# huangnengCSU/NanoSNP

Hardware: AMD Instinct MI355X
Metric: candidate SNP sites/sec (pileup encode + model fwd), 30x windows (higher is better)
Workload: dtype f32; 1 GPU; BASELINE configs[1]: pileup encode + PileupModel fwd, 1M synthetic 30x windows (G2) resident in HBM, batch=4096; batch=4096, windows_resident_per_gpu=1048576, streams=32, precision=fp32, parallelism=site-sharded x1, rooted gather of calls, world_size_observed=1, gather=torch

## Files before the change

### nanosnp_amd/csrc/nsnp_api.hip

```cpp
#include "nsnp_common.hpp"

#include <new>

extern "C" int nsnp_version(void) { return 101; }

extern "C" const char* nsnp_strerror(int code)
{
    switch (code) {
    case NSNP_OK: return "ok";
    case NSNP_EINVAL: return "invalid argument";
    case NSNP_ENOMEM: return "out of memory";
    case NSNP_EHIP: return "HIP runtime error";
    case NSNP_ENOWEIGHTS: return "weights not loaded";
    case NSNP_EARCH: return "device is not gfx950";
    case NSNP_ESHAPE: return "unsupported model dimensions";
    case NSNP_ENOTSUP: return "optional component unavailable (RCCL not found)";
    case NSNP_ECOMM: return "RCCL call failed";
    default: return "unknown error";
    }
}

static hipError_t g_create_err = hipSuccess;

extern "C" int nsnp_last_hip_error(const nsnp_ctx* ctx, const char** text)
{
    const hipError_t e = ctx ? ctx->last_err : g_create_err;
    if (text) *text = hipGetErrorString(e);
    return (int)e;
}

extern "C" int nsnp_ctx_create(int device, nsnp_ctx** out)
{
    if (!out) return NSNP_EINVAL;
    *out = nullptr;
    nsnp_ctx* ctx = new (std::nothrow) nsnp_ctx();
    if (!ctx) return NSNP_ENOMEM;
    memset((void*)ctx, 0, sizeof(*ctx));
    ctx->device = device;
    ctx->last_err = hipSuccess;
    ctx->chunk_sites = 32768;
    ctx->hap_chunk = 16384;
    ctx->precision = 0;
    ctx->hap_precision = 0;
    ctx->cat_precision = 0;
    ctx->cat_conv_lds = 1;
    ctx->cat_conv_pix2 = 1;
    ctx->hap_b3x = 1;
    ctx->tok_fused = 0;
    ctx->proj1_tiles = 4;
    ctx->fused_l1 = 1;
    ctx->l0_rs = 2;
    ctx->l1_rs = 1;
    ctx->l1_stagger = 0;
    ctx->head_rs = 1;
    ctx->rs_prio = 0;
    hipDeviceProp_t prop;
    hipError_t e = hipSetDevice(device);
    if (e == hipSuccess) e = hipGetDeviceProperties(&prop, device);
    if (e != hipSuccess) { g_create_err = e; delete ctx; return NSNP_EHIP; }
    if (strncmp(prop.gcnArchName, "gfx950", 6) != 0) { delete ctx; return NSNP_EARCH; }
    ctx->n_cu = prop.multiProcessorCount;
    *out = ctx;
    return NSNP_OK;
}

void nsnp_hap_free(nsnp_ctx* ctx);
int  nsnp_hap_reserve(nsnp_ctx* ctx);
void nsnp_cat_free(nsnp_ctx* ctx);
void nsnp_tok_free(nsnp_ctx* ctx);

constexpr size_t TIMER_MAX_PAIRS = 8192;

ScopedKernelTimer::ScopedKernelTimer(nsnp_ctx* c, int kernel, hipStream_t stream)
    : ctx(c), k(kernel), s(stream), stop_ev(nullptr), on(false)
{
    KernelTimer* t = c->timer;
    if (!t || !t->enabled || t->used[k] >= TIMER_MAX_PAIRS) return;
    if (t->used[k] == t->start[k].size()) {
        hipEvent_t a, b;
        if (hipEventCreate(&a) != hipSuccess) return;
        if (hipEventCreate(&b) != hipSuccess) { (void)hipEventDestroy(a); return; }
        t->start[k].push_back(a); t->stop[k].push_back(b);
    }
    const size_t i = t->used[k]++;
    (void)hipEventRecord(t->start[k][i], s);
    stop_ev = t->stop[k][i];
    on = true;
}
void ScopedKernelTimer::stop() { if (on) { (void)hipEventRecord(stop_ev, s); on = false; } }
ScopedKernelTimer::~ScopedKernelTimer() { stop(); }

extern "C" int nsnp_ctx_set_option(nsnp_ctx* ctx, const char* name, int64_t value)
{
    if (!ctx || !name) return NSNP_EINVAL;
    if (strcmp(name, "cat_precision") == 0) {
        if (value != 0 && value != 1 && value != 2) return NSNP_EINVAL;
        ctx->cat_precision = (int)value;
        return NSNP_OK;
    }
    if (strcmp(name, "tok_fused") == 0) {
        if (value != 0 && value != 1) return NSNP_EINVAL;
        ctx->tok_fused = (int)value;
        return NSNP_OK;
    }
    if (strcmp(name, "hap_b3x") == 0) {
        if (value != 0 && value != 1) return NSNP_EINVAL;
        ctx->hap_b3x = (int)value;
        return NSNP_OK;
    }
    if (strcmp(name, "cat_conv_pix2") == 0) {
        if (value != 0 && value != 1) return NSNP_EINVAL;
        ctx->cat_conv_pix2 = (int)value;
        return NSNP_OK;
    }
    if (strcmp(name, "cat_conv_lds") == 0) {
        if (value != 0 && value != 1) return NSNP_EINVAL;
        ctx->cat_conv_lds = (int)value;
        return NSNP_OK;
    }
    if (strcmp(name, "hap_precision") == 0) {
        if (value != 0 && value != 1 && value != 2) return NSNP_EINVAL;
        ctx->hap_precision = (int)value;
        return nsnp_hap_reserve(ctx);
    }
    if (strcmp(name, "hap_pass_sites") == 0) {
        if (value < 128 || value > 131072 || value % 128) return NSNP_EINVAL;
        const int64_t old = ctx->hap_chunk;
        ctx->hap_chunk = value;
        const int rc = nsnp_hap_reserve(ctx);
        if (rc) { ctx->hap_chunk = old; (void)nsnp_hap_reserve(ctx); }
        return rc;
    }
    if (strcmp(name, "pileup_precision") == 0) {
        if (value != 0 && value != 1 && value != 2) return NSNP_EINVAL;
        ctx->precision = (int)value;
        if (value == 2 && ctx->ws_h0 && ctx->ws_h0_floats < 192) return nsnp_ctx_reserve(ctx, ctx->chunk_sites);
        return NSNP_OK;
    }
    if (strcmp(name, "fused_l1") == 0) {
        if (value != 0 && value != 1) return NSNP_EINVAL;
        ctx->fused_l1 = (int)value;
        return NSNP_OK;
    }
    if (strcmp(name, "l0_register_stationary") == 0) {
        if (value != 0 && value != 1 && value != 2) return NSNP_EINVAL;
        ctx->l0_rs = (int)value;
        return NSNP_OK;
    }
    if (strcmp(name, "l1_register_stationary") == 0) {
        if (value != 0 && value != 1 && value != 2) return NSNP_EINVAL;
        ctx->l1_rs = (int)value;
        return NSNP_OK;
    }
    if (strcmp(name, "l0_input_weights_in_lds") == 0) {
        if (value != 0 && value != 1) return NSNP_EINVAL;
        ctx->l0_wx_lds = (int)value;
        return NSNP_OK;
    }
    if (strcmp(name, "static_priority") == 0) {
        if (value < 0 || value > 3) return NSNP_EINVAL;
        ctx->rs_prio = (int)value;
        return NSNP_OK;
    }
    if (strcmp(name, "head_split") == 0) {
        if (value != 0 && value != 1) return NSNP_EINVAL;
        ctx->head_rs = (int)value;
        return NSNP_OK;
    }
    if (strcmp(name, "l1_stagger") == 0) {
        if (value != 0 && value != 1) return NSNP_EINVAL;
        ctx->l1_stagger = (int)value;
        return NSNP_OK;
    }
    if (strcmp(name, "l1_site_groups") == 0) {
        if (value != 0 && value != 1 && value != 2 && value != 4) return NSNP_EINVAL;
        ctx->l1_rs_groups = (int)value;
        return NSNP_OK;
    }
    if (strcmp(name, "l0_site_groups") == 0) {
        if (value != 0 && value != 1 && value != 2 && value != 4) return NSNP_EINVAL;
        ctx->l0_rs_groups = (int)value;
        return NSNP_OK;
    }
    if (strcmp(name, "fused_waves") == 0) {
        if (value != 0 && value != 4 && value != 8 && value != 12) return NSNP_EINVAL;
        ctx->fused_waves = (int)value;
        return NSNP_OK;
    }
    if (strcmp(name, "proj1_tiles") == 0) {
        if (value < 1 || value > 64) return NSNP_EINVAL;
        ctx->proj1_tiles = (int)value;
        return NSNP_OK;
    }
    if (strcmp(name, "recurrence_waves") == 0) {
        if (value != 0 && value != 1 && value != 2 && value != 4 && value != 8) return NSNP_EINVAL;
        ctx->force_wpb = (int)value;
        return NSNP_OK;
    }
    return NSNP_EINVAL;
}

extern "C" int nsnp_ctx_enable_timing(nsnp_ctx* ctx, int enable)
{
    if (!ctx) return NSNP_EINVAL;
    if (!ctx->timer) {
        ctx->timer = new (std::nothrow) KernelTimer();
        if (!ctx->timer) return NSNP_ENOMEM;
        for (int k = 0; k < NSNP_K_COUNT; ++k) ctx->timer->used[k] = 0;
    }
    ctx->timer->enabled = enable != 0;
    return NSNP_OK;
}

extern "C" int nsnp_ctx_read_timing(nsnp_ctx* ctx, int kernel, double* total_ms, int64_t* launches)
{
    if (!ctx || kernel < 0 || kernel >= NSNP_K_COUNT || !total_ms || !launches) return NSNP_EINVAL;
    *total_ms = 0.0; *launches = 0;
    KernelTimer* t = ctx->timer;
    if (!t) return NSNP_OK;
    for (size_t i = 0; i < t->used[kernel]; ++i) {
        NSNP_HIP(ctx, hipEventSynchronize(t->stop[kernel][i]));
        float ms = 0.f;
        NSNP_HIP(ctx, hipEventElapsedTime(&ms, t->start[kernel][i], t->stop[kernel][i]));
        *total_ms += ms; ++*launches;
    }
    t->used[kernel] = 0;
    return NSNP_OK;
}

static void free_ws(nsnp_ctx* ctx)
{
    if (ctx->ws_h0) (void)hipFree(ctx->ws_h0);
    if (ctx->ws_xp1) (void)hipFree(ctx->ws_xp1);
    if (ctx->ws_h1c) (void)hipFree(ctx->ws_h1c);
    ctx->ws_h0 = ctx->ws_xp1 = ctx->ws_h1c = nullptr;
    ctx->ws_h0_floats = 0;
}

extern "C" int nsnp_ctx_destroy(nsnp_ctx* ctx)
{
    if (!ctx) return NSNP_EINVAL;
    (void)hipSetDevice(ctx->device);
    (void)hipDeviceSynchronize();
    free_ws(ctx);
    if (ctx->pw.arena) (void)hipFree(ctx->pw.arena);
    if (ctx->pw16.arena) (void)hipFree(ctx->pw16.arena);
    if (ctx->pw16.l1f_bias) (void)hipFree(ctx->pw16.l1f_bias);
    if (ctx->pwb3.arena) (void)hipFree(ctx->pwb3.arena);
    if (ctx->sel_tmp) (void)hipFree(ctx->sel_tmp);
    if (ctx->fil_tmp) (void)hipFree(ctx->fil_tmp);
    if (ctx->rec_tmp) (void)hipFree(ctx->rec_tmp);
    if (ctx->lab_tmp) (void)hipFree(ctx->lab_tmp);
    nsnp_tok_free(ctx);
    (void)nsnp_comm_destroy(ctx);
// ... 110 lines not shown
```

### nanosnp_amd/csrc/nsnp_common.hpp

```cpp
#pragma once

#include <hip/hip_runtime.h>
#include <stdint.h>
#include <stdlib.h>
#include <string.h>
#include <vector>

#include "nanosnp.h"

typedef float f32x4 __attribute__((ext_vector_type(4)));
typedef int   i32x4 __attribute__((ext_vector_type(4)));

#define NSNP_CDIV(a, b) (((a) + (b) - 1) / (b))

constexpr int PW = NSNP_PILEUP_WINDOW;
constexpr int PC = NSNP_PILEUP_CHANNELS;
constexpr int PH = 64;
constexpr int PG = 4 * PH;
constexpr int PCENTER = 16;
constexpr int PSTEPS1 = PCENTER + 1;


struct PileupWeightsDev {
    float* l0_whh[2];
    float* l0_wih[2];
    float* l0_wlast[2];
    void*  l0_wx[2];
    float* l1_wih[2];
    float* l1_bias[2];
    float* l1_bias_raw[2];
    float* l1_whh[2];
    float* proj_w;
    float* proj_b;
    float* dense_w;
    float* dense_b;
    float* head_w;
    float* head_b;
    float* arena;
    size_t arena_bytes;
    bool   loaded;
};

struct PileupWeightsF16 {
    void* l0_whh[2]; void* l0_wih_hi[2]; void* l0_wih_lo[2]; void* l1_wih[2]; void* l1_whh[2];
    void* l1f_hi[2]; void* l1f_lo[2]; float* l1f_bias;
    void* l0_wih_rs[2];
    void* l1_wih_rs[2]; void* l1_whh_rs[2];
    void* l0_whh_rs[2];
    void* proj_w; void* dense_w; void* head_w;
    void* arena; size_t arena_bytes; bool loaded;
};

struct PileupWeightsB3 {
    void* l0_whh[2]; void* l0_wih[2]; void* l1_wih[2]; void* l1_whh[2];
    void* proj_w; void* dense_w; void* head_w;
    float* proj_b; float* dense_b; float* head_b;
    void* arena; size_t arena_bytes; bool loaded;
};

struct HapWeightsDev;
struct CatWeightsDev;

enum { NSNP_K_L0 = 0, NSNP_K_PROJ1, NSNP_K_L1, NSNP_K_HEAD, NSNP_K_ENCODE, NSNP_K_HAPFEAT, NSNP_K_HAPLSTM, NSNP_K_CATCONV, NSNP_K_CAT,
       NSNP_K_COUNT };
struct KernelTimer {
    std::vector<hipEvent_t> start[NSNP_K_COUNT], stop[NSNP_K_COUNT];
    size_t used[NSNP_K_COUNT];
    bool enabled;
};

struct PostOut { uint8_t* gt_arg; uint8_t* zy_arg; float* gt_max; float* zy_max; };

struct nsnp_ctx {
    int device;
    int n_cu;
    hipError_t last_err;
    bool attr_set;
    bool attr_set_f16;
    bool attr_set_b3;
    int hap_b3x;
    int cat_conv_pix2;
    int cat_conv_lds;
    int cat_precision;
    int hap_precision;
    int precision;
    int fused_waves;
    int l0_rs;
    int l1_rs_groups;
    int l1_rs;
    int l0_rs_groups;
    int fused_l1;
    int proj1_tiles;
    int force_wpb;
    int l0_wx_lds;
    int rs_prio;
    int head_rs;
    int l1_stagger;
    int64_t chunk_sites;
    float*  ws_h0;
    int     ws_h0_floats;
    float*  ws_xp1;
    float*  ws_h1c;
    PileupWeightsDev pw;
    PileupWeightsF16 pw16;
    PileupWeightsB3 pwb3;
    HapWeightsDev* hw;
    void*  hap_ws; size_t hap_ws_bytes; int64_t hap_ws_chunk;
    int64_t hap_chunk;
    CatWeightsDev* cw;
    void*  cat_ws; size_t cat_ws_bytes;
    int64_t* sel_tmp; size_t sel_tmp_bytes;
    int64_t* fil_tmp; size_t fil_tmp_bytes;
    void* rec_tmp; size_t rec_tmp_bytes;
    void* lab_tmp; size_t lab_tmp_bytes;
    void* tok_ws; size_t tok_ws_bytes;
    void* ctg_ws; size_t ctg_ws_bytes;
    int tok_fused;
    bool af_cached; uint64_t af_bits, af_t; int af_k, af_mode; uint32_t af_table_words[128];
    bool af2_cached; uint64_t af2_bits, af2_t; int af2_k, af2_mode; uint32_t af2_table_words[128];
    KernelTimer* timer;
    void* comm; int comm_rank, comm_world;
    bool comm_borrowed;
};

struct ScopedKernelTimer {
    nsnp_ctx* ctx; int k; hipStream_t s; hipEvent_t stop_ev; bool on;
    ScopedKernelTimer(nsnp_ctx* c, int kernel, hipStream_t stream);
    void stop();
    ~ScopedKernelTimer();
};

#define NSNP_HIP(ctx, call)                                                        \
    do {                                                                           \
        hipError_t e_ = (call);                                                    \
        if (e_ != hipSuccess) { (ctx)->last_err = e_; return NSNP_EHIP; }          \
    } while (0)

typedef float (*nsnp_wfun)(const void* user, int row, int k);
void nsnp_pack_image(float* img, int n_tiles, int n_j4, nsnp_wfun f, const void* user);

int nsnp_ctx_need_xp1(nsnp_ctx* ctx);

int nsnp_pileup_forward_impl(nsnp_ctx* ctx, const int32_t* x, const int64_t* center_idx,
                             int64_t N, float* gt, float* zy, const PostOut* post, bool* post_written, hipStream_t s);
int nsnp_pileup_pack_weights(nsnp_ctx* ctx, const float* const* w);
int nsnp_pileup_forward_f16x3(nsnp_ctx* ctx, const int32_t* x, const int64_t* center_idx,
                              int64_t N, float* gt, float* zy, hipStream_t s);
int nsnp_pileup_pack_weights_f16(nsnp_ctx* ctx, const float* const* w);
int nsnp_pileup_forward_bf16x3(nsnp_ctx* ctx, const int32_t* x, const int64_t* center_idx, int64_t N, float* gt, float* zy,
                               const PostOut* post, hipStream_t s);
int nsnp_pileup_pack_weights_bf16(nsnp_ctx* ctx, const float* const* w);
```

### nanosnp_amd/csrc/nsnp_lstm_cell.hpp

```cpp
#pragma once

namespace nsnp_cell {

constexpr float LOG2E = 1.4426950408889634f;

static inline float lstm_gate_scale(int R) { return (R & 3) == 2 ? -2.0f * LOG2E : -LOG2E; }

__device__ __forceinline__ float cap64(float z) { return __builtin_amdgcn_fmed3f(z, -3.0e38f, 64.0f); }

__device__ __forceinline__ float lstm_cell(float zi, float zf, float zg, float zo, float c_prev, float& c_new)
{
    const float ei = __builtin_amdgcn_exp2f(zi);
    const float ef = __builtin_amdgcn_exp2f(zf);
    const float eo = __builtin_amdgcn_exp2f(zo);
    const float eg = __builtin_amdgcn_exp2f(cap64(zg));
    constexpr float K = -2.0f * LOG2E;
    const float tg = 1.0f + eg;
    const float ig = __builtin_fmaf(-K, eg, K) * __builtin_amdgcn_rcpf(__builtin_fmaf(ei, tg, tg));
    const float fg = __builtin_amdgcn_rcpf(1.0f + ef);
    const float cn = __builtin_fmaf(fg, c_prev, ig);
    const float ec = __builtin_amdgcn_exp2f(cap64(cn));
    c_new = cn;
    const float tc = 1.0f + ec;
    return (1.0f - ec) * __builtin_amdgcn_rcpf(__builtin_fmaf(eo, tc, tc));
}

}
```

### nanosnp_amd/csrc/pileup_forward.hip

```cpp
#include "nsnp_common.hpp"
#include "nsnp_lstm_cell.hpp"
#include "nsnp_devclock.hpp"
#include "nsnp_bf16.hpp"
#include <type_traits>

namespace {

constexpr float LOG2E = 1.4426950408889634f;

__device__ __forceinline__ f32x4 mfma4(float a, float b, f32x4 c)
{
    return __builtin_amdgcn_mfma_f32_16x16x4f32(a, b, c, 0, 0, 0);
}
__device__ __forceinline__ float sigmoid_f(float x)
{
    return __builtin_amdgcn_rcpf(1.0f + __builtin_amdgcn_exp2f(-LOG2E * x));
}
__device__ __forceinline__ float tanh_f(float x)
{
    return __builtin_fmaf(-2.0f, __builtin_amdgcn_rcpf(1.0f + __builtin_amdgcn_exp2f((2.0f * LOG2E) * x)), 1.0f);
}

__device__ __forceinline__ float lstm_cell(float zi, float zf, float zg, float zo, float& c)
{
// ... 770 lines not shown
        for (int k = 0; k < 2 * NSG; ++k) {
            const int64_t site = base_site + (tid >> 5) + 8 * k;
            const int64_t sc = site < N ? site : N - 1;
            sreg[k] = *reinterpret_cast<const f32x4*>(H0 + (sc * PW + t) * 128 + 4 * cid);
        }
    };
    auto store_h0 = [&](int buf) {
#pragma unroll
        for (int k = 0; k < 2 * NSG; ++k)
            *reinterpret_cast<f32x4*>(h0s + ((size_t)buf * NS + (tid >> 5) + 8 * k) * RS_H0ROW + 4 * slot) = sreg[k];
    };
    load_h0(dir ? PW - 1 : 0);
    store_h0(0);
    if (PSTEPS1 > 1) load_h0(dir ? PW - 2 : 1);
    __syncthreads();

    float c[NSG][4];
#pragma unroll
    for (int sg = 0; sg < NSG; ++sg)
#pragma unroll
        for (int u = 0; u < 4; ++u) c[sg][u] = 0.f;

    for (int s = 0; s < PSTEPS1; ++s) {
        const int t = dir ? PW - 1 - s : s;
        const int cur = s & 1;
        const float* h0b = h0s + (size_t)cur * NS * RS_H0ROW;
        const float* hrb = h1x + (size_t)(cur ^ 1) * NS * RS_XROW;
        float* hwb = h1x + (size_t)cur * NS * RS_XROW;
#pragma unroll
        for (int sg = 0; sg < NSG; ++sg) {
            const float* r0 = h0b + (size_t)(16 * sg + n) * RS_H0ROW + 4 * q;
            f32x4 acc[4];
#pragma unroll
            for (int u = 0; u < 4; ++u) acc[u] = lbias[(4 * wave + u) * 4 + q];
#pragma unroll
            for (int j = 0; j < 8; ++j) {
                if (sg == 0 && j == 2 && s + 1 < PSTEPS1) {
                    __builtin_amdgcn_sched_barrier(0);
                    store_h0(cur ^ 1);
                    __builtin_amdgcn_sched_barrier(0);
                }
                if (sg == 0 && j == 5 && s + 2 < PSTEPS1) {
                    __builtin_amdgcn_sched_barrier(0);
                    load_h0(dir ? t - 2 : t + 2);
                    __builtin_amdgcn_sched_barrier(0);
                }
                const f32x4 b4 = *reinterpret_cast<const f32x4*>(r0 + 64 * (j >> 2) + 16 * (j & 3));
#pragma unroll
                for (int e = 0; e < 4; ++e)
#pragma unroll
                    for (int u = 0; u < 4; ++u) acc[u] = mfma4(Wih[u][j][e], b4[e], acc[u]);
            }
            if (s > 0) {
                const float* r1 = hrb + (size_t)(16 * sg + n) * RS_XROW + 4 * q;
#pragma unroll
                for (int j = 0; j < 4; ++j) {
                    const f32x4 b4 = *reinterpret_cast<const f32x4*>(r1 + 16 * j);
#pragma unroll
                    for (int e = 0; e < 4; ++e)
#pragma unroll
                        for (int u = 0; u < 4; ++u) acc[u] = mfma4(Whh[u][j][e], b4[e], acc[u]);
                }
            }
            f32x4 hn;
#pragma unroll
            for (int u = 0; u < 4; ++u) {
                hn[u] = lstm_cell(acc[u][0], acc[u][1], acc[u][2], acc[u][3], c[sg][u]);
            }
            *reinterpret_cast<f32x4*>(hwb + (size_t)(16 * sg + n) * RS_XROW + 16 * wave + 4 * q) = hn;
        }
        lds_barrier();
    }
    const float* hfin = h1x + (size_t)((PSTEPS1 - 1) & 1) * NS * RS_XROW;
#pragma unroll
    for (int sg = 0; sg < NSG; ++sg) {
        const int64_t site = base_site + 16 * sg + n;
        if (site < N)
            *reinterpret_cast<f32x4*>(H1c + site * 128 + dir * 64 + q * 16 + 4 * wave) =
                *reinterpret_cast<const f32x4*>(hfin + (size_t)(16 * sg + n) * RS_XROW + 16 * wave + 4 * q);
    }
    NSNP_DEVCLK_STOP(1)
}

__global__ __launch_bounds__(256) void k_pileup_head(
    const float* __restrict__ H1c, int64_t N,
    const float* __restrict__ proj_w, const float* __restrict__ proj_b,
    const float* __restrict__ dense_w, const float* __restrict__ dense_b,
    const float* __restrict__ head_w, const float* __restrict__ head_b,
    float* __restrict__ gt_prob, float* __restrict__ zy_prob)
{
    const int tid = threadIdx.x, lane = tid & 63, wave = tid >> 6;
    const int q = lane >> 4;
    const int64_t site = ((int64_t)blockIdx.x * 4 + wave) * 16 + (lane & 15);
    const bool live = site < N;
    const int64_t sc = live ? site : N - 1;
    const f32x4* __restrict__ hin = reinterpret_cast<const f32x4*>(H1c + sc * 128 + q * 16);
    float b[32];
#pragma unroll
    for (int v = 0; v < 4; ++v) {
        const f32x4 a = hin[v], bb = hin[16 + v];
#pragma unroll
        for (int e = 0; e < 4; ++e) { b[4 * v + e] = a[e]; b[16 + 4 * v + e] = bb[e]; }
    }
    f32x4 ap[8];
    {
        const f32x4* pb = reinterpret_cast<const f32x4*>(proj_b);
#pragma unroll
        for (int i = 0; i < 8; ++i) ap[i] = pb[i * 64 + lane];
        wave_gemm<8, 8, 0, 8>(reinterpret_cast<const f32x4*>(proj_w), lane, b, ap);
    }
    float b2[32];
#pragma unroll
    for (int i = 0; i < 8; ++i)
#pragma unroll
        for (int g = 0; g < 4; ++g) b2[4 * i + g] = ap[i][g];
    f32x4 ad[16];
    {
        const f32x4* db = reinterpret_cast<const f32x4*>(dense_b);
#pragma unroll
        for (int i = 0; i < 16; ++i) ad[i] = db[i * 64 + lane];
        wave_gemm<16, 8, 0, 8>(reinterpret_cast<const f32x4*>(dense_w), lane, b2, ad);
    }
    float b3[64];
#pragma unroll
    for (int i = 0; i < 16; ++i)
#pragma unroll
        for (int g = 0; g < 4; ++g) b3[4 * i + g] = tanh_f(ad[i][g]);
    f32x4 ah[2];
    {
        const f32x4* hb = reinterpret_cast<const f32x4*>(head_b);
        ah[0] = hb[lane]; ah[1] = hb[64 + lane];
        wave_gemm2x16(reinterpret_cast<const f32x4*>(head_w), lane, b3, ah);
    }
    const float NEG = -3.0e38f;
    float g0[4], g1[4];
#pragma unroll
    for (int g = 0; g < 4; ++g) {
        g0[g] = ah[0][g];
        const bool is_gt = (q == 0) || (q == 1 && g == 0);
        g1[g] = is_gt ? ah[1][g] : NEG;
    }
    float mx = fmaxf(fmaxf(fmaxf(g0[0], g0[1]), fmaxf(g0[2], g0[3])), fmaxf(fmaxf(g1[0], g1[1]), fmaxf(g1[2], g1[3])));
    mx = fmaxf(mx, __shfl_xor(mx, 16));
    mx = fmaxf(mx, __shfl_xor(mx, 32));
    float e0[4], e1[4], sum = 0.f;
#pragma unroll
    for (int g = 0; g < 4; ++g) {
        e0[g] = __expf(g0[g] - mx);
        e1[g] = g1[g] > -1.0e38f ? __expf(g1[g] - mx) : 0.f;
        sum += e0[g] + e1[g];
    }
    sum += __shfl_xor(sum, 16);
    sum += __shfl_xor(sum, 32);
    const float z1 = ah[1][1], z2 = ah[1][2], z3 = ah[1][3];
    const float zm = fmaxf(z1, fmaxf(z2, z3));
    const float ez1 = __expf(z1 - zm), ez2 = __expf(z2 - zm), ez3 = __expf(z3 - zm);
    const float zs = ez1 + ez2 + ez3;
    if (live) {
        float* gp = gt_prob + site * NSNP_GT_CLASSES;
#pragma unroll
        for (int g = 0; g < 4; ++g) gp[4 * q + g] = e0[g] / sum;
        if (q == 0) {
#pragma unroll
            for (int g = 0; g < 4; ++g) gp[16 + g] = e1[g] / sum;
        }
        if (q == 1) {
// ... 235 lines not shown
    for (int t = 0; t < 16; ++t) {
        const int layer = t / 8, kind = t % 4;
        const size_t cols = kind == 0 ? (layer ? 2 * PH : PC) : (kind == 1 ? PH : 1);
        scaled[t].resize((size_t)4 * PH * cols);
        for (int r = 0; r < 4 * PH; ++r) {
            const float f = (r / PH == 2) ? -2.0f * LOG2E : -LOG2E;
            for (size_t k = 0; k < cols; ++k) scaled[t][r * cols + k] = f * w[t][r * cols + k];
        }
        ws[t] = scaled[t].data();
    }
    for (int d = 0; d < 2; ++d) {
        const float* const* l0 = ws + d * 4;
        const float* const* l1 = ws + 8 + d * 4;
        MatRef m;
        m = MatRef{l0[1], PH, nullptr, nullptr};  nsnp_pack_image(h_l0_whh[d], 16, 4, f_whh, &m);
        m = MatRef{l0[0], PC, nullptr, nullptr};  nsnp_pack_image(h_l0_wih[d], 16, 1, f_wih0, &m);
        for (int tile = 0; tile < 16; ++tile)
            for (int lane = 0; lane < 64; ++lane) {
                const int tr = gate_row(16 * tile + (lane & 15)), kq = lane >> 4;
                float v = 0.f;
                if (kq < 2) v = l0[0][tr * PC + 16 + kq];
                else if (kq == 2) v = l0[2][tr] + l0[3][tr];
                h_l0_wlast[d][tile * 64 + lane] = v;
            }
        pack_b3(reinterpret_cast<uint16_t*>(h_l0_wx[d]), 16, 1, [&](int row, int, int q, int j) {
            const int k = 8 * q + j, tr = gate_row(row);
            return k < PC ? l0[0][tr * PC + k] : (k == PC ? l0[2][tr] + l0[3][tr] : 0.f);
        });
        m = MatRef{l1[0], 2 * PH, nullptr, nullptr};  nsnp_pack_image(h_l1_wih[d], 16, 8, f_wih1, &m);
        for (int tile = 0; tile < 16; ++tile)
            for (int lane = 0; lane < 64; ++lane)
                for (int g = 0; g < 4; ++g) {
                    const int tr = gate_row(16 * tile + 4 * (lane >> 4) + g);
                    h_l1_b[d][(tile * 64 + lane) * 4 + g] = l1[2][tr] + l1[3][tr];
                    h_l1_braw[d][(tile * 64 + lane) * 4 + g] = w[8 + d * 4 + 2][tr] + w[8 + d * 4 + 3][tr];
                }
        m = MatRef{l1[1], PH, nullptr, nullptr};  nsnp_pack_image(h_l1_whh[d], 16, 4, f_whh, &m);
    }
    {
        MatRef m{w[16], 128, nullptr, nullptr};  nsnp_pack_image(h_proj, 8, 8, f_proj, &m);
        for (int tile = 0; tile < 8; ++tile) for (int lane = 0; lane < 64; ++lane) for (int g = 0; g < 4; ++g)
            h_pb[(tile * 64 + lane) * 4 + g] = w[17][16 * tile + 4 * (lane >> 4) + g];
        MatRef md{w[18], 128, nullptr, nullptr}; nsnp_pack_image(h_dense, 16, 8, f_dense, &md);
        for (int tile = 0; tile < 16; ++tile) for (int lane = 0; lane < 64; ++lane) for (int g = 0; g < 4; ++g)
            h_db[(tile * 64 + lane) * 4 + g] = w[19][16 * tile + 4 * (lane >> 4) + g];
        HeadRef hr{w[20], w[22]};  nsnp_pack_image(h_head, 2, 16, f_head, &hr);
        for (int tile = 0; tile < 2; ++tile) for (int lane = 0; lane < 64; ++lane) for (int g = 0; g < 4; ++g) {
            const int row = 16 * tile + 4 * (lane >> 4) + g;
            h_hb[(tile * 64 + lane) * 4 + g] = row < 21 ? w[21][row] : (row < 24 ? w[23][row - 21] : 0.f);
        }
    }
    if (pw.arena && pw.arena_bytes != total * sizeof(float)) { (void)hipFree(pw.arena); pw.arena = nullptr; }
    if (!pw.arena) {
        NSNP_HIP(ctx, hipMalloc((void**)&pw.arena, total * sizeof(float)));
        pw.arena_bytes = total * sizeof(float);
    }
    NSNP_HIP(ctx, hipMemcpy(pw.arena, host.data(), total * sizeof(float), hipMemcpyHostToDevice));
    auto dev = [&](const float* hp) { return pw.arena + (hp - host.data()); };
    for (int d = 0; d < 2; ++d) {
        pw.l0_whh[d] = dev(h_l0_whh[d]); pw.l0_wih[d] = dev(h_l0_wih[d]); pw.l0_wlast[d] = dev(h_l0_wlast[d]);
        pw.l0_wx[d] = dev(h_l0_wx[d]);
        pw.l1_wih[d] = dev(h_l1_wih[d]); pw.l1_bias[d] = dev(h_l1_b[d]); pw.l1_bias_raw[d] = dev(h_l1_braw[d]); pw.l1_whh[d] = dev(h_l1_whh[d]);
    }
    pw.proj_w = dev(h_proj); pw.proj_b = dev(h_pb); pw.dense_w = dev(h_dense); pw.dense_b = dev(h_db);
    pw.head_w = dev(h_head); pw.head_b = dev(h_hb);
    pw.loaded = true;
    return NSNP_OK;
}

static int set_lds_attr_once(nsnp_ctx* ctx)
{
    if (ctx->attr_set) return NSNP_OK;
    NSNP_HIP(ctx, hipFuncSetAttribute((const void*)k_pileup_l0<8>, hipFuncAttributeMaxDynamicSharedMemorySize, L0_LDS_BYTES));
    NSNP_HIP(ctx, hipFuncSetAttribute((const void*)k_pileup_l0<4>, hipFuncAttributeMaxDynamicSharedMemorySize, L0_LDS_BYTES));
    NSNP_HIP(ctx, hipFuncSetAttribute((const void*)k_pileup_l0<2>, hipFuncAttributeMaxDynamicSharedMemorySize, L0_LDS_BYTES));
    NSNP_HIP(ctx, hipFuncSetAttribute((const void*)k_pileup_l0<1>, hipFuncAttributeMaxDynamicSharedMemorySize, L0_LDS_BYTES));
    NSNP_HIP(ctx, hipFuncSetAttribute((const void*)k_pileup_proj1, hipFuncAttributeMaxDynamicSharedMemorySize, P1_LDS_BYTES));
    NSNP_HIP(ctx, hipFuncSetAttribute((const void*)k_pileup_l1<8>, hipFuncAttributeMaxDynamicSharedMemorySize, L1_LDS_BYTES));
    NSNP_HIP(ctx, hipFuncSetAttribute((const void*)k_pileup_l1<4>, hipFuncAttributeMaxDynamicSharedMemorySize, L1_LDS_BYTES));
    NSNP_HIP(ctx, hipFuncSetAttribute((const void*)k_pileup_l1<2>, hipFuncAttributeMaxDynamicSharedMemorySize, L1_LDS_BYTES));
    NSNP_HIP(ctx, hipFuncSetAttribute((const void*)k_pileup_l1<1>, hipFuncAttributeMaxDynamicSharedMemorySize, L1_LDS_BYTES));
    NSNP_HIP(ctx, hipFuncSetAttribute((const void*)k_pileup_l1_rs4<1>, hipFuncAttributeMaxDynamicSharedMemorySize, rs4_l1_lds_bytes(1)));
    NSNP_HIP(ctx, hipFuncSetAttribute((const void*)k_pileup_l1_rs4<2>, hipFuncAttributeMaxDynamicSharedMemorySize, rs4_l1_lds_bytes(2)));
    NSNP_HIP(ctx, hipFuncSetAttribute((const void*)k_pileup_l1_rs32<4, true>, hipFuncAttributeMaxDynamicSharedMemorySize, rs32_l1_lds_bytes(4)));
    NSNP_HIP(ctx, hipFuncSetAttribute((const void*)k_pileup_l1_rs32<2, true>, hipFuncAttributeMaxDynamicSharedMemorySize, rs32_l1_lds_bytes(2)));
    NSNP_HIP(ctx, hipFuncSetAttribute((const void*)k_pileup_l1_rs32<4, false>, hipFuncAttributeMaxDynamicSharedMemorySize, rs32_l1_lds_bytes(4)));
    NSNP_HIP(ctx, hipFuncSetAttribute((const void*)k_pileup_l1_rs32<2, false>, hipFuncAttributeMaxDynamicSharedMemorySize, rs32_l1_lds_bytes(2)));
    ctx->attr_set = true;
    return NSNP_OK;
}

int nsnp_pileup_forward_impl(nsnp_ctx* ctx, const int32_t* x, const int64_t* center_idx,
                             int64_t N, float* gt, float* zy, const PostOut* post, bool* post_written, hipStream_t s)
{
    if (!ctx->pw.loaded) return NSNP_ENOWEIGHTS;
    if (N == 0) return NSNP_OK;
    int rc = set_lds_attr_once(ctx);
    if (rc) return rc;
    if (!ctx->ws_h0) { rc = nsnp_ctx_reserve(ctx, ctx->chunk_sites); if (rc) return rc; }
    const PileupWeightsDev& pw = ctx->pw;
    for (int64_t base = 0; base < N; base += ctx->chunk_sites) {
        const int64_t n = (N - base < ctx->chunk_sites) ? N - base : ctx->chunk_sites;
        const int32_t* xc = center_idx ? x : x + base * (PW * PC);
        const int64_t* cc = center_idx ? center_idx + base : nullptr;
        const int64_t waves_total = NSNP_CDIV(n, 16) * 2;
        int wpb = 8;
        while (wpb > 1 && waves_total / wpb < (int64_t)ctx->n_cu / 2) wpb >>= 1;
        if (ctx->force_wpb) wpb = ctx->force_wpb;
        const dim3 g_rec((unsigned)NSNP_CDIV(n, 16 * wpb), 2);
        if (ctx->l0_rs == 2) {
            ScopedKernelTimer tm(ctx, NSNP_K_L0, s);
            hipLaunchKernelGGL(k_pileup_l0_rsx, dim3((unsigned)NSNP_CDIV(n, 16), 2), dim3(256), 0, s, xc, cc, n,
                               pw.l0_whh[0], pw.l0_whh[1], (const __bf16*)pw.l0_wx[0], (const __bf16*)pw.l0_wx[1], ctx->ws_h0);
        } else if (ctx->l0_rs) {
            ScopedKernelTimer tm(ctx, NSNP_K_L0, s);
            int nsg = 1;
            if (ctx->l0_rs_groups) nsg = ctx->l0_rs_groups;
#define LAUNCH_RS(G) hipLaunchKernelGGL(k_pileup_l0_rs32<G>, dim3((unsigned)NSNP_CDIV(n, 16 * G), 2), dim3(256), 0, s, xc, cc, n, \
                           pw.l0_whh[0], pw.l0_whh[1], pw.l0_wih[0], pw.l0_wih[1], pw.l0_wlast[0], pw.l0_wlast[1], ctx->ws_h0)
            if (ctx->l0_wx_lds && nsg == 1)
                hipLaunchKernelGGL((k_pileup_l0_rs32<1, true>), dim3((unsigned)NSNP_CDIV(n, 16), 2), dim3(256), 0, s, xc, cc, n,
                                   pw.l0_whh[0], pw.l0_whh[1], pw.l0_wih[0], pw.l0_wih[1], pw.l0_wlast[0], pw.l0_wlast[1], ctx->ws_h0);
            else
            if (nsg == 4) LAUNCH_RS(4); else if (nsg == 2) LAUNCH_RS(2); else LAUNCH_RS(1);
#undef LAUNCH_RS
        } else
        { ScopedKernelTimer tm(ctx, NSNP_K_L0, s);
#define LAUNCH_L0(W) hipLaunchKernelGGL(k_pileup_l0<W>, g_rec, dim3(64 * W), L0_LDS_BYTES, s, xc, cc, n, \
                           pw.l0_whh[0], pw.l0_whh[1], pw.l0_wih[0], pw.l0_wih[1], pw.l0_wlast[0], pw.l0_wlast[1], ctx->ws_h0)
        if (wpb == 8) LAUNCH_L0(8); else if (wpb == 4) LAUNCH_L0(4); else if (wpb == 2) LAUNCH_L0(2); else LAUNCH_L0(1);
#undef LAUNCH_L0
        }
        if (ctx->l1_rs == 1) {
            ScopedKernelTimer tm(ctx, NSNP_K_L1, s);
            int g1 = 1;
            if (ctx->l1_rs_groups == 1 || ctx->l1_rs_groups == 2) g1 = ctx->l1_rs_groups;
#define LAUNCH_R4(G) hipLaunchKernelGGL(k_pileup_l1_rs4<G>, dim3((unsigned)NSNP_CDIV(n, 16 * G), 2), dim3(256), rs4_l1_lds_bytes(G), s, \
                           ctx->ws_h0, n, pw.l1_wih[0], pw.l1_wih[1], pw.l1_whh[0], pw.l1_whh[1], pw.l1_bias[0], pw.l1_bias[1], ctx->ws_h1c)
            if (g1 == 2) LAUNCH_R4(2); else LAUNCH_R4(1);
#undef LAUNCH_R4
        } else if (ctx->l1_rs == 2) {
            ScopedKernelTimer tm(ctx, NSNP_K_L1, s);
            int g1 = NSNP_CDIV(n, 64) * 2 >= (int64_t)ctx->n_cu ? 4 : 2;
            if (ctx->l1_rs_groups) g1 = ctx->l1_rs_groups;
#define LAUNCH_R1(G) hipLaunchKernelGGL((k_pileup_l1_rs32<G, ST>), dim3((unsigned)NSNP_CDIV(n, 16 * G), 2), dim3(512), rs32_l1_lds_bytes(G), s, \
                           ctx->ws_h0, n, pw.l1_wih[0], pw.l1_wih[1], pw.l1_whh[0], pw.l1_whh[1], pw.l1_bias[0], pw.l1_bias[1], ctx->ws_h1c)
            if (ctx->l1_stagger) { constexpr bool ST = true; if (g1 == 4) LAUNCH_R1(4); else LAUNCH_R1(2); }
            else { constexpr bool ST = false; if (g1 == 4) LAUNCH_R1(4); else LAUNCH_R1(2); }
#undef LAUNCH_R1
        } else {
        { const int rx = nsnp_ctx_need_xp1(ctx); if (rx) return rx; }
        const int64_t n_rt = NSNP_CDIV(n * PSTEPS1, 16);
        int64_t gp = NSNP_CDIV(n_rt, 16 * (int64_t)ctx->proj1_tiles);
        if (gp > ctx->n_cu) gp = ctx->n_cu;
        if (gp < 1) gp = 1;
        { ScopedKernelTimer tm(ctx, NSNP_K_PROJ1, s);
        hipLaunchKernelGGL(k_pileup_proj1, dim3((unsigned)gp, 2), dim3(1024), P1_LDS_BYTES, s, ctx->ws_h0, n,
                           pw.l1_wih[0], pw.l1_wih[1], pw.l1_bias[0], pw.l1_bias[1], ctx->ws_xp1); }
        { ScopedKernelTimer tm(ctx, NSNP_K_L1, s);
#define LAUNCH_L1(W) hipLaunchKernelGGL(k_pileup_l1<W>, g_rec, dim3(64 * W), L1_LDS_BYTES, s, ctx->ws_xp1, n, \
                           pw.l1_whh[0], pw.l1_whh[1], ctx->ws_h1c)
        if (wpb == 8) LAUNCH_L1(8); else if (wpb == 4) LAUNCH_L1(4); else if (wpb == 2) LAUNCH_L1(2); else LAUNCH_L1(1);
#undef LAUNCH_L1
        }
        }
        ScopedKernelTimer tm_head(ctx, NSNP_K_HEAD, s);
        if (ctx->head_rs) {
            int64_t gh = NSNP_CDIV(n, 16);
            if (gh > 2 * (int64_t)ctx->n_cu) gh = 2 * (int64_t)ctx->n_cu;
            const PostOut po = post ? *post : PostOut{nullptr, nullptr, nullptr, nullptr};
            hipLaunchKernelGGL(k_pileup_head_rs, dim3((unsigned)gh), dim3(512), 0, s, ctx->ws_h1c, n,
                               pw.proj_w, pw.proj_b, pw.dense_w, pw.dense_b, pw.head_w, pw.head_b,
                               gt + base * NSNP_GT_CLASSES, zy + base * NSNP_ZY_CLASSES,
                               po.gt_arg ? po.gt_arg + base : nullptr, po.gt_arg ? po.zy_arg + base : nullptr,
                               po.gt_arg ? po.gt_max + base : nullptr, po.gt_arg ? po.zy_max + base : nullptr);
            if (post_written) *post_written = po.gt_arg != nullptr;
        } else
        hipLaunchKernelGGL(k_pileup_head, dim3((unsigned)NSNP_CDIV(n, 64)), dim3(256), 0, s, ctx->ws_h1c, n,
                           pw.proj_w, pw.proj_b, pw.dense_w, pw.dense_b, pw.head_w, pw.head_b,
                           gt + base * NSNP_GT_CLASSES, zy + base * NSNP_ZY_CLASSES);
    }
    NSNP_HIP(ctx, hipGetLastError());
    return NSNP_OK;
}

NSNP_DEVCLK_READER(nsnp_devclk_read_pileup)

extern "C" int nsnp_pileup_postprocess(nsnp_ctx* ctx, const float* gt_prob, const float* zy_prob,
                                       const int32_t* x, int64_t N, uint8_t* gt_arg, uint8_t* zy_arg,
                                       float* gt_max, float* zy_max, int32_t* depth, void* stream)
{
    if (!ctx || N < 0 || (N > 0 && (!gt_prob || !zy_prob || !gt_arg || !zy_arg || !gt_max || !zy_max || (depth && !x)))) return NSNP_EINVAL;
    if (N == 0) return NSNP_OK;
    hipLaunchKernelGGL(k_pileup_post, dim3((unsigned)NSNP_CDIV(N, 256)), dim3(256), 0, (hipStream_t)stream,
                       gt_prob, zy_prob, x, N, gt_arg, zy_arg, gt_max, zy_max, depth);
    NSNP_HIP(ctx, hipGetLastError());
    return NSNP_OK;
}
```

Baseline: 20.54 million sites/s.

## Add woven L1 LSTM kernel overlapping next-step projection with cell math

```diff
diff --git a/nanosnp_amd/csrc/nsnp_api.hip b/nanosnp_amd/csrc/nsnp_api.hip
--- a/nanosnp_amd/csrc/nsnp_api.hip
+++ b/nanosnp_amd/csrc/nsnp_api.hip
@@ -52,6 +52,7 @@
     ctx->l0_rs = 2;
     ctx->l1_rs = 1;
     ctx->l1_stagger = 0;
+    ctx->l1_weave = 1;
     ctx->head_rs = 1;
     ctx->rs_prio = 0;
     hipDeviceProp_t prop;
@@ -170,6 +171,11 @@
     if (strcmp(name, "l1_stagger") == 0) {
         if (value != 0 && value != 1) return NSNP_EINVAL;
         ctx->l1_stagger = (int)value;
+        return NSNP_OK;
+    }
+    if (strcmp(name, "l1_weave") == 0) {
+        if (value != 0 && value != 1) return NSNP_EINVAL;
+        ctx->l1_weave = (int)value;
         return NSNP_OK;
     }
     if (strcmp(name, "l1_site_groups") == 0) {
diff --git a/nanosnp_amd/csrc/nsnp_common.hpp b/nanosnp_amd/csrc/nsnp_common.hpp
--- a/nanosnp_amd/csrc/nsnp_common.hpp
+++ b/nanosnp_amd/csrc/nsnp_common.hpp
@@ -96,6 +96,7 @@
     int rs_prio;
     int head_rs;
     int l1_stagger;
+    int l1_weave;
     int64_t chunk_sites;
     float*  ws_h0;
     int     ws_h0_floats;
diff --git a/nanosnp_amd/csrc/nsnp_lstm_cell.hpp b/nanosnp_amd/csrc/nsnp_lstm_cell.hpp
--- a/nanosnp_amd/csrc/nsnp_lstm_cell.hpp
+++ b/nanosnp_amd/csrc/nsnp_lstm_cell.hpp
@@ -25,4 +25,45 @@
     return (1.0f - ec) * __builtin_amdgcn_rcpf(__builtin_fmaf(eo, tc, tc));
 }
 
+struct CellSlices { float ei[4], ef[4], eo[4], eg[4], t[4], d[4], m[4], fg[4]; };
+constexpr int CELL_SLICES = 80;
+
+template <int I, typename Z4>
+__device__ __forceinline__ void lstm_cell_slice(CellSlices& w, const Z4 (&z)[4], float (&c)[4], Z4& h)
+{
+    static_assert(I >= 0 && I < CELL_SLICES, "slice index");
+    constexpr int st = I >> 2, u = I & 3;
+    constexpr float K = -2.0f * LOG2E;
+    if constexpr (st == 0) w.ei[u] = __builtin_amdgcn_exp2f(z[u][0]);
+    else if constexpr (st == 1) w.ef[u] = __builtin_amdgcn_exp2f(z[u][1]);
+    else if constexpr (st == 2) w.eo[u] = __builtin_amdgcn_exp2f(z[u][3]);
+    else if constexpr (st == 3) w.t[u] = cap64(z[u][2]);
+    else if constexpr (st == 4) w.eg[u] = __builtin_amdgcn_exp2f(w.t[u]);
+    else if constexpr (st == 5) w.t[u] = 1.0f + w.eg[u];
+    else if constexpr (st == 6) w.d[u] = __builtin_fmaf(w.ei[u], w.t[u], w.t[u]);
+    else if constexpr (st == 7) w.d[u] = __builtin_amdgcn_rcpf(w.d[u]);
+    else if constexpr (st == 8) w.m[u] = __builtin_fmaf(-K, w.eg[u], K);
+    else if constexpr (st == 9) w.m[u] = w.m[u] * w.d[u];
+    else if constexpr (st == 10) w.fg[u] = 1.0f + w.ef[u];
+    else if constexpr (st == 11) w.fg[u] = __builtin_amdgcn_rcpf(w.fg[u]);
+    else if constexpr (st == 12) c[u] = __builtin_fmaf(w.fg[u], c[u], w.m[u]);
+    else if constexpr (st == 13) w.t[u] = cap64(c[u]);
+    else if constexpr (st == 14) w.eg[u] = __builtin_amdgcn_exp2f(w.t[u]);
+    else if constexpr (st == 15) w.t[u] = 1.0f + w.eg[u];
+    else if constexpr (st == 16) w.d[u] = __builtin_fmaf(w.eo[u], w.t[u], w.t[u]);
+    else if constexpr (st == 17) w.d[u] = __builtin_amdgcn_rcpf(w.d[u]);
+    else if constexpr (st == 18) w.m[u] = 1.0f - w.eg[u];
+    else h[u] = w.m[u] * w.d[u];
+    if constexpr (st == 0) asm volatile("" : "+v"(w.ei[u]));
+    else if constexpr (st == 1) asm volatile("" : "+v"(w.ef[u]));
+    else if constexpr (st == 2) asm volatile("" : "+v"(w.eo[u]));
+    else if constexpr (st == 4 || st == 14) asm volatile("" : "+v"(w.eg[u]));
+    else if constexpr (st == 3 || st == 5 || st == 13 || st == 15) asm volatile("" : "+v"(w.t[u]));
+    else if constexpr (st == 6 || st == 7 || st == 16 || st == 17) asm volatile("" : "+v"(w.d[u]));
+    else if constexpr (st == 8 || st == 9 || st == 18) asm volatile("" : "+v"(w.m[u]));
+    else if constexpr (st == 10 || st == 11) asm volatile("" : "+v"(w.fg[u]));
+    else if constexpr (st == 12) asm volatile("" : "+v"(c[u]));
+    else { float v = h[u]; asm volatile("" : "+v"(v)); h[u] = v; }
 }
+
+}
diff --git a/nanosnp_amd/csrc/pileup_forward.hip b/nanosnp_amd/csrc/pileup_forward.hip
--- a/nanosnp_amd/csrc/pileup_forward.hip
+++ b/nanosnp_amd/csrc/pileup_forward.hip
@@ -876,6 +876,186 @@
     NSNP_DEVCLK_STOP(1)
 }
 
+constexpr int rs4w_l1_lds_bytes() { return rs4_l1_lds_bytes(1) + 4 * 4 * 2 * 64 * 16; }
+
+template <int... I, class F>
+__device__ __forceinline__ void static_for_seq(std::integer_sequence<int, I...>, F&& f) { (f(std::integral_constant<int, I>{}), ...); }
+template <int N, class F>
+__device__ __forceinline__ void static_for(F&& f) { static_for_seq(std::make_integer_sequence<int, N>{}, f); }
+
+template <int CELL_PER_GAP, int CELL_FIRST_GAP>
+__global__ __launch_bounds__(256, 2) void k_pileup_l1_rs4w(
+    const float* __restrict__ H0, int64_t N,
+    const float* __restrict__ wih0, const float* __restrict__ wih1,
+    const float* __restrict__ whh0, const float* __restrict__ whh1,
+    const float* __restrict__ bias0, const float* __restrict__ bias1,
+    float* __restrict__ H1c)
+{
+    extern __shared__ f32x4 lds[];
+    float* const h0s = reinterpret_cast<float*>(lds);
+    float* const h1x = h0s + 2 * 16 * RS_H0ROW;
+    f32x4* const lbias = reinterpret_cast<f32x4*>(h1x + 2 * 16 * RS_XROW);
+    f32x4* const lwhh = lbias + 64;
+    const int dir = blockIdx.y;
+    const int tid = threadIdx.x, lane = tid & 63, wave = tid >> 6;
+    const int n = lane & 15, q = lane >> 4;
+    NSNP_DEVCLK_START
+    const int64_t base_site = (int64_t)blockIdx.x * 16;
+
+    f32x4 Wih[4][8], Whh[4][2];
+    f32x4* const lw = lwhh + wave * (4 * 2 * 64) + lane;
+    {
+        const f32x4* __restrict__ gih = reinterpret_cast<const f32x4*>(dir ? wih1 : wih0);
+        const f32x4* __restrict__ ghh = reinterpret_cast<const f32x4*>(dir ? whh1 : whh0);
+#pragma unroll
+        for (int u = 0; u < 4; ++u) {
+#pragma unroll
+            for (int j = 0; j < 8; ++j) Wih[u][j] = gih[((4 * wave + u) * 8 + j) * 64 + lane];
+#pragma unroll
+            for (int j = 0; j < 2; ++j) Whh[u][j] = ghh[((4 * wave + u) * 4 + j) * 64 + lane];
+#pragma unroll
+            for (int j = 0; j < 2; ++j) lw[(2 * u + j) * 64] = ghh[((4 * wave + u) * 4 + 2 + j) * 64 + lane];
+        }
+        if (tid < 64) lbias[tid] = reinterpret_cast<const f32x4*>(dir ? bias1 : bias0)[(tid >> 2) * 64 + 16 * (tid & 3)];
+    }
+
+    const int cid = tid & 31;
+    const int slot = (cid & 16) + 4 * (cid & 3) + ((cid >> 2) & 3);
+    f32x4 sreg[2];
+    const float* const h0wg = H0 + base_site * (PW * 128);
+    unsigned hoff[2];
+#pragma unroll
+    for (int k = 0; k < 2; ++k) {
+        const int64_t site = base_site + (tid >> 5) + 8 * k;
+        const int64_t sc = site < N ? site : N - 1;
+        hoff[k] = (unsigned)((int)(sc - base_site) * (PW * 128) + 4 * cid) * 4u;
+    }
+    auto tpos = [&](int u) { return dir ? PW - 1 - u : u; };
+    auto load_h0 = [&](int t) {
+#pragma unroll
+        for (int k = 0; k < 2; ++k) {
+            asm volatile("" : "+v"(hoff[k]));
+            sreg[k] = *reinterpret_cast<const f32x4*>(reinterpret_cast<const char*>(h0wg + t * 128) + hoff[k]);
+        }
+    };
+    auto store_h0 = [&](int buf) {
+#pragma unroll
+        for (int k = 0; k < 2; ++k)
+            *reinterpret_cast<f32x4*>(h0s + ((size_t)buf * 16 + (tid >> 5) + 8 * k) * RS_H0ROW + 4 * slot) = sreg[k];
+    };
+    static_assert(PSTEPS1 >= 3, "the pipeline stages three steps in its prologue");
+    load_h0(tpos(0)); store_h0(0);
+    load_h0(tpos(1)); store_h0(1);
+    __syncthreads();
+    load_h0(tpos(2));
+
+    float c[4];
+#pragma unroll
+    for (int u = 0; u < 4; ++u) c[u] = 0.f;
+
+    auto project_reads = [&](int buf, f32x4 (&p)[4], f32x4& b0) __attribute__((always_inline)) {
+        b0 = *reinterpret_cast<const f32x4*>(h0s + ((size_t)buf * 16 + n) * RS_H0ROW + 4 * q);
+#pragma unroll
+        for (int u = 0; u < 4; ++u) p[u] = lbias[(4 * wave + u) * 4 + q];
+    };
+    auto project = [&](int buf, f32x4 (&p)[4], const f32x4& b0, auto cell_tag, f32x4 (&a)[4], float* hout, int tnext)
+                       __attribute__((always_inline)) {
+        constexpr bool CELL = decltype(cell_tag)::value;
+        constexpr int NGAPS = (nsnp_cell::CELL_SLICES + CELL_PER_GAP - 1) / CELL_PER_GAP, CELL_END = CELL_FIRST_GAP + NGAPS;
+        static_assert(CELL_END + 8 <= 128, "the cell, the h1 row and the h0 staging end inside the burst");
+        const float* r0 = h0s + ((size_t)buf * 16 + n) * RS_H0ROW + 4 * q;
+        f32x4 b4[2];
+        b4[0] = b0;
+        nsnp_cell::CellSlices w;
+        f32x4 hn;
+        static_for<128>([&](auto gc) __attribute__((always_inline)) {
+            constexpr int g = decltype(gc)::value, j = g >> 4, e = (g >> 2) & 3, u = g & 3;
+            if constexpr ((g & 15) == 0 && j + 1 < 8)
+                b4[(j + 1) & 1] = *reinterpret_cast<const f32x4*>(r0 + 64 * ((j + 1) >> 2) + 16 * ((j + 1) & 3));
+            p[u] = mfma4(Wih[u][j][e], b4[j & 1][e], p[u]);
+            if constexpr (CELL) {
+                static_for<CELL_PER_GAP>([&](auto kc) __attribute__((always_inline)) {
+                    constexpr int i = (g - CELL_FIRST_GAP) * CELL_PER_GAP + decltype(kc)::value;
+                    if constexpr (g >= CELL_FIRST_GAP && i < nsnp_cell::CELL_SLICES) nsnp_cell::lstm_cell_slice<i>(w, a, c, hn);
+                });
+                if constexpr (g == CELL_END) *reinterpret_cast<f32x4*>(hout) = hn;
+                if constexpr (g == CELL_END + 2) store_h0(buf ^ 1);
+                if constexpr (g == CELL_END + 4) load_h0(tnext);
+            }
+            __builtin_amdgcn_sched_barrier(0);
+        });
+    };
+
+    f32x4 accA[4], accB[4], bfirst;
+    project_reads(0, accA, bfirst);
+    project(0, accA, bfirst, std::false_type{}, accA, nullptr, 0);
+    lds_barrier();
+
+    auto step = [&](int s, f32x4 (&acc)[4], f32x4 (&nxt)[4], auto first_tag, auto last_tag) __attribute__((always_inline)) {
+        constexpr bool FIRST = decltype(first_tag)::value, LAST = decltype(last_tag)::value;
+        const int cur = s & 1;
+        float* const hw = h1x + ((size_t)cur * 16 + n) * RS_XROW + 16 * wave + 4 * q;
+        f32x4 b0;
+        if constexpr (!FIRST) {
+            const float* r1 = h1x + ((size_t)(cur ^ 1) * 16 + n) * RS_XROW + 4 * q;
+            f32x4 hb0 = *reinterpret_cast<const f32x4*>(r1), hb1 = *reinterpret_cast<const f32x4*>(r1 + 16), A2[4], A3[4];
+#define RS4W_KBLOCK(A, HB)                                                                             \
+            _Pragma("unroll") for (int e = 0; e < 4; ++e)                                              \
+                _Pragma("unroll") for (int u = 0; u < 4; ++u) acc[u] = mfma4(A[e], HB[e], acc[u]);
+#pragma unroll
+            for (int u = 0; u < 4; ++u) A2[u] = lw[(2 * u) * 64];
+            __builtin_amdgcn_sched_barrier(0);
+            RS4W_KBLOCK(Whh[u][0], hb0)
+            __builtin_amdgcn_sched_barrier(0);
+            hb0 = *reinterpret_cast<const f32x4*>(r1 + 32);
+#pragma unroll
+            for (int u = 0; u < 4; ++u) A3[u] = lw[(2 * u + 1) * 64];
+            RS4W_KBLOCK(Whh[u][1], hb1)
+            __builtin_amdgcn_sched_barrier(0);
+            hb1 = *reinterpret_cast<const f32x4*>(r1 + 48);
+            RS4W_KBLOCK(A2[u], hb0)
+            __builtin_amdgcn_sched_barrier(0);
+            if constexpr (!LAST) project_reads(cur ^ 1, nxt, b0);
+            RS4W_KBLOCK(A3[u], hb1)
+            __builtin_amdgcn_sched_barrier(0);
+#undef RS4W_KBLOCK
+        } else {
+            project_reads(cur ^ 1, nxt, b0);
+            __builtin_amdgcn_sched_barrier(0);
+        }
+        if constexpr (!LAST) {
+            project(cur ^ 1, nxt, b0, std::true_type{}, acc, hw, tpos(s + 3 < PSTEPS1 ? s + 3 : PSTEPS1 - 1));
+        } else {
+            f32x4 hn;
+#pragma unroll
+            for (int u = 0; u < 4; ++u) hn[u] = lstm_cell(acc[u][0], acc[u][1], acc[u][2], acc[u][3], c[u]);
+            *reinterpret_cast<f32x4*>(hw) = hn;
+        }
+        lds_barrier();
+    };
+    static_assert(PSTEPS1 % 2 == 1, "the step loop is unrolled by two");
+    step(0, accA, accB, std::true_type{}, std::false_type{});
+    for (int s = 1; s < PSTEPS1 - 2; s += 2) {
+        step(s, accB, accA, std::false_type{}, std::false_type{});
+        step(s + 1, accA, accB, std::false_type{}, std::false_type{});
+    }
+    step(PSTEPS1 - 2, accB, accA, std::false_type{}, std::false_type{});
+    step(PSTEPS1 - 1, accA, accB, std::false_type{}, std::true_type{});
+
+    const int64_t site = base_site + n;
+    if (site < N)
+        *reinterpret_cast<f32x4*>(H1c + site * 128 + dir * 64 + q * 16 + 4 * wave) =
+            *reinterpret_cast<const f32x4*>(h1x + ((size_t)((PSTEPS1 - 1) & 1) * 16 + n) * RS_XROW + 16 * wave + 4 * q);
+    NSNP_DEVCLK_STOP(1)
+}
+#ifndef RS4W_PER_GAP
+#define RS4W_PER_GAP 80
+#endif
+#ifndef RS4W_FIRST_GAP
+#define RS4W_FIRST_GAP 0
+#endif
+static_assert(rs4w_l1_lds_bytes() <= 80 * 1024, "two workgroups per CU");
+
 __global__ __launch_bounds__(256) void k_pileup_head(
     const float* __restrict__ H1c, int64_t N,
     const float* __restrict__ proj_w, const float* __restrict__ proj_b,
@@ -1277,6 +1457,7 @@
     NSNP_HIP(ctx, hipFuncSetAttribute((const void*)k_pileup_l1<1>, hipFuncAttributeMaxDynamicSharedMemorySize, L1_LDS_BYTES));
     NSNP_HIP(ctx, hipFuncSetAttribute((const void*)k_pileup_l1_rs4<1>, hipFuncAttributeMaxDynamicSharedMemorySize, rs4_l1_lds_bytes(1)));
     NSNP_HIP(ctx, hipFuncSetAttribute((const void*)k_pileup_l1_rs4<2>, hipFuncAttributeMaxDynamicSharedMemorySize, rs4_l1_lds_bytes(2)));
+    NSNP_HIP(ctx, hipFuncSetAttribute((const void*)k_pileup_l1_rs4w<RS4W_PER_GAP, RS4W_FIRST_GAP>, hipFuncAttributeMaxDynamicSharedMemorySize, rs4w_l1_lds_bytes()));
     NSNP_HIP(ctx, hipFuncSetAttribute((const void*)k_pileup_l1_rs32<4, true>, hipFuncAttributeMaxDynamicSharedMemorySize, rs32_l1_lds_bytes(4)));
     NSNP_HIP(ctx, hipFuncSetAttribute((const void*)k_pileup_l1_rs32<2, true>, hipFuncAttributeMaxDynamicSharedMemorySize, rs32_l1_lds_bytes(2)));
     NSNP_HIP(ctx, hipFuncSetAttribute((const void*)k_pileup_l1_rs32<4, false>, hipFuncAttributeMaxDynamicSharedMemorySize, rs32_l1_lds_bytes(4)));
@@ -1332,7 +1513,12 @@
             if (ctx->l1_rs_groups == 1 || ctx->l1_rs_groups == 2) g1 = ctx->l1_rs_groups;
 #define LAUNCH_R4(G) hipLaunchKernelGGL(k_pileup_l1_rs4<G>, dim3((unsigned)NSNP_CDIV(n, 16 * G), 2), dim3(256), rs4_l1_lds_bytes(G), s, \
                            ctx->ws_h0, n, pw.l1_wih[0], pw.l1_wih[1], pw.l1_whh[0], pw.l1_whh[1], pw.l1_bias[0], pw.l1_bias[1], ctx->ws_h1c)
-            if (g1 == 2) LAUNCH_R4(2); else LAUNCH_R4(1);
+            if (g1 == 2) LAUNCH_R4(2);
+            else if (ctx->l1_weave)
+                hipLaunchKernelGGL((k_pileup_l1_rs4w<RS4W_PER_GAP, RS4W_FIRST_GAP>), dim3((unsigned)NSNP_CDIV(n, 16), 2), dim3(256),
+                                   rs4w_l1_lds_bytes(), s, ctx->ws_h0, n, pw.l1_wih[0], pw.l1_wih[1], pw.l1_whh[0], pw.l1_whh[1],
+                                   pw.l1_bias[0], pw.l1_bias[1], ctx->ws_h1c);
+            else LAUNCH_R4(1);
 #undef LAUNCH_R4
         } else if (ctx->l1_rs == 2) {
             ScopedKernelTimer tm(ctx, NSNP_K_L1, s);
```

After: 20.80 million sites/s, median of 6. 1.01x the previous value.
